# HarryShomer/LPFormer

Hardware: AMD Instinct MI355X
Metric: candidate link-pairs scored/sec (whole node) (higher is better)
Workload: dtype f32

## Files before the change

lpformer_amd/csrc/tail_chain.hip:

```cpp
#include <type_traits>

#include "lpf_common.h"

namespace {

typedef float f32x4 __attribute__((ext_vector_type(4)));

#ifndef LPF_TC_GROUPS
#define LPF_TC_GROUPS 4
#endif
constexpr int TC_GROUPS = LPF_TC_GROUPS;
constexpr int TC_WAVES = 2 * TC_GROUPS;
constexpr int TC_THREADS = 64 * TC_WAVES;

struct TailArgs {
    int64_t M;
    const float *x; int64_t ldx; int KA;
    const float *addend; int64_t ldadd;
    const float *wA, *lnA_g, *lnA_b; int NA;
    const float *tail; int64_t ldtail;
    const float *wB, *bB, *lnB_g, *lnB_b; int NB;
    const float *re; int64_t ldre;
    const float *wC, *bC; int NC;
    const float *wdot, *bdot;
    float *logit, *prob;
    const float *part;
    const float *bnd;
    int64_t units_cap;
    const int32_t *type_ptr;
    const float *att_bias;
    const int64_t *sel_ctl;
    int n_counts;
    const float *rows; int64_t ldrows;
    const int32_t *perm;
    const int64_t *n_full;
    const float *bC_empty;
    const float *row_empty;
    const float *X; int64_t ldX;
    const int64_t *batch; int64_t batch_ld, n_rows;
    const float *wE, *bE, *lnE_g, *lnE_b;
};

constexpr int tc_per_thread(int ntp) { return (ntp * 64 + TC_THREADS - 1) / TC_THREADS; }
constexpr int tc_stage_stride(int ntp) { return (ntp * 64 + 511) / 512 * 512; }

typedef short bf16x4_bits __attribute__((ext_vector_type(4)));
template <int P, int NTP, typename T>
__device__ __forceinline__ void tc_load(T (&r)[P], const float *packed, int stage, int tid) {
    const T *src = reinterpret_cast<const T *>(packed) + (int64_t)stage * tc_stage_stride(NTP);
#pragma unroll
    for (int e = 0; e < P; ++e) {
        const int i = e * TC_THREADS + tid;
#ifdef TC_NOWLOAD
        r[e] = T{};
        (void)src; (void)i;
#else
        r[e] = src[i < tc_stage_stride(NTP) ? i : 0];
#endif
    }
}
template <int P, typename T>
__device__ __forceinline__ void tc_store(const T (&r)[P], T *slab, int tid) {
#pragma unroll
    for (int e = 0; e < P; ++e) slab[e * TC_THREADS + tid] = r[e];
}

#define TC_PIN() __builtin_amdgcn_sched_barrier(0)

template <int TPW>
__device__ __forceinline__ void tc_mfma(f32x4 (&acc)[TPW], const f32x4 *lw, const f32x4 bv, bool last = true) {
    f32x4 a[TPW];
#pragma unroll
    for (int c = 0; c < TPW; ++c) a[c] = lw[c * 64];
#pragma unroll
    for (int u = 0; u < 4; ++u) {
#pragma unroll
        for (int c = 0; c < TPW - 1; ++c) acc[c] = __builtin_amdgcn_mfma_f32_16x16x4f32(a[c][u], bv[u], acc[c], 0, 0, 0);
        if (last) acc[TPW - 1] = __builtin_amdgcn_mfma_f32_16x16x4f32(a[TPW - 1][u], bv[u], acc[TPW - 1], 0, 0, 0);
    }
}
template <int TPW>
__device__ __forceinline__ void tc_mfma(f32x4 (&acc)[TPW], const uint2 *lw, const f32x4 bv, bool last = true) {
    bf16x4_bits b;
#pragma unroll
    for (int u = 0; u < 4; ++u) b[u] = (short)lpf_f32_to_bf16(bv[u]);
#pragma unroll
    for (int c = 0; c < TPW; ++c) {
        if (c == TPW - 1 && !last) break;
        const uint2 w = lw[c * 64];
        const bf16x4_bits a = {(short)(w.x & 0xffffu), (short)(w.x >> 16), (short)(w.y & 0xffffu), (short)(w.y >> 16)};
        acc[c] = __builtin_amdgcn_mfma_f32_16x16x16bf16_1k(a, b, acc[c], 0, 0, 0);
    }
}

constexpr int TC_XCH_SLOT = TC_WAVES * 16;
template <int TPW>
__device__ __forceinline__ void tc_layernorm(f32x4 (&acc)[TPW], int fbase, int n, const float *g, const float *b, int half,
                                             int q, float *my_x, const float *peer_x, bool relu) {
    float s1 = 0.f;
#pragma unroll
    for (int c = 0; c < TPW; ++c) s1 += acc[c][0] + acc[c][1] + acc[c][2] + acc[c][3];
    s1 = lpf_quad_sum(s1);
    if (q == 0) *my_x = s1;
    __syncthreads();
    const float mean = (half == 0 ? s1 + *peer_x : *peer_x + s1) / (float)n;
    float s2 = 0.f;
#pragma unroll
    for (int c = 0; c < TPW; ++c)
#pragma unroll
        for (int r = 0; r < 4; ++r) {
            const float d = (fbase + 16 * c + r < n) ? acc[c][r] - mean : 0.f;
            s2 += d * d;
        }
    s2 = lpf_quad_sum(s2);
    if (q == 0) my_x[TC_XCH_SLOT] = s2;
    __syncthreads();
    const float p2 = peer_x[TC_XCH_SLOT];
    const float rstd = 1.0f / sqrtf((half == 0 ? s2 + p2 : p2 + s2) / (float)n + 1e-5f);
#pragma unroll
    for (int c = 0; c < TPW; ++c) {
        const f32x4 gg = *reinterpret_cast<const f32x4 *>(g + fbase + 16 * c);
        const f32x4 bb = *reinterpret_cast<const f32x4 *>(b + fbase + 16 * c);
        acc[c] = (acc[c] - mean) * rstd * gg + bb;
        if (relu) {
#pragma unroll
            for (int r = 0; r < 4; ++r) acc[c][r] = fmaxf(acc[c][r], 0.f);
        }
    }
}

#ifdef TC_STAMPS
__device__ uint64_t *tc_stamp_buf = nullptr;
#define TC_STAMP(k) do { if (lane == 0) st_t[k] = wall_clock64(); } while (0)
#define TC_STAMPS_OUT(kind) do { if (lane == 0 && tc_stamp_buf) { uint64_t *o__ = tc_stamp_buf + ((int64_t)blockIdx.x * TC_WAVES + wave) * 16; \
        for (int k__ = 0; k__ < 8; ++k__) o__[k__] = st_t[k__]; o__[15] = (kind); } } while (0)
#else
#define TC_STAMP(k) do { } while (0)
#define TC_STAMPS_OUT(kind) do { } while (0)
#endif

template <int NTA, int NTB, int NTC>
struct TcShape {
    static constexpr int NTPA = (NTA + 1) & ~1, NTPB = (NTB + 1) & ~1, NTPC = (NTC + 1) & ~1;
    static constexpr int PA = tc_per_thread(NTPA), PB = tc_per_thread(NTPB), PC = tc_per_thread(NTPC);
    static constexpr int PM = PA > PB ? (PA > PC ? PA : PC) : (PB > PC ? PB : PC);
    static constexpr int SLAB = PM * TC_THREADS;
    static constexpr int HT = NTPA > NTPB ? NTPA : NTPB;
    static constexpr int HID = TC_GROUPS * HT * 64;
    static constexpr int XCH = 5 * TC_WAVES * 16;
    static constexpr int VEC_B = 3 * 16 * NTPA, VEC_C = VEC_B + 3 * 16 * NTPB, VEC_N = VEC_C + 2 * 16 * NTPC;
    static constexpr size_t BYTES = (size_t)(2 * SLAB + HID) * sizeof(f32x4) + (XCH + VEC_N) * sizeof(float);
    static_assert(NTC >= 32 || BYTES <= 81920, "two workgroups share a CU's 160 KB of LDS");
};

template <int NTA, int NTB, int NTC, int WM = 0, bool ROWS = false, bool EW = false>
__global__ __launch_bounds__(TC_THREADS, NTC >= 32 ? 2 : (TC_THREADS >= 512 ? 4 : 3)) void tail_chain_kernel(const TailArgs A) {
    using S = TcShape<NTA, NTB, NTC>;
    constexpr bool WB = WM != 0;
    using WT = typename std::conditional<WM == 1, uint2, f32x4>::type;
    constexpr int NTPA = S::NTPA, NTPB = S::NTPB, NTPC = S::NTPC;
    constexpr int TPWA = NTPA / 2, TPWB = NTPB / 2, TPWC = NTPC / 2;
    constexpr int NGE = NTA;
    extern __shared__ __attribute__((aligned(16))) f32x4 lds[];
    f32x4 *hid = lds + 2 * S::SLAB;
    float *xch = reinterpret_cast<float *>(hid + S::HID);
    const int tid = threadIdx.x, lane = tid & 63, wave = tid >> 6;
    const int grp = wave >> 1, half = wave & 1, q = lane >> 4, j = lane & 15;
    float *my_x = xch + wave * 16 + j;
    const float *peer_x = xch + (wave ^ 1) * 16 + j;
    float *vec = xch + S::XCH;
    f32x4 *my_hid = hid + (grp * S::HT) * 64 + lane;
    int buf = 0;
#ifdef TC_STAMPS
    uint64_t st_t[8] = {0};
    TC_STAMP(0);
#endif

    const int64_t tile = blockIdx.x;
    const int64_t pos = tile * (16 * TC_GROUPS) + grp * 16 + j;
    const bool live = pos < A.M;
    bool lite = false;
    int64_t m = pos;
    if constexpr (ROWS) {
        if (A.perm) {
            m = A.perm[live ? pos : A.M - 1];
            lite = tile * (16 * TC_GROUPS) >= *A.n_full;
        }
    }
    const int64_t mm = live ? m : (ROWS && A.perm ? m : A.M - 1);
    bool no_sel = false;
    if constexpr (ROWS) no_sel = A.perm && A.row_empty && (live ? pos : A.M - 1) >= *A.n_full;

    constexpr int VP0 = EW ? 0 : S::VEC_B / 4, VPN = S::VEC_N / 4 - VP0, VPT = (VPN + TC_THREADS - 1) / TC_THREADS;
    f32x4 vecr[VPT];
#pragma unroll
    for (int e = 0; e < VPT; ++e) {
        int p = VP0 + e * TC_THREADS + tid;
        p = p < S::VEC_N / 4 ? p : S::VEC_N / 4 - 1;
        const float *src;
        if (p >= S::VEC_C / 4) {
            const int o = p - S::VEC_C / 4;
            src = o < 4 * NTPC ? (lite ? A.bC_empty : A.bC) + 4 * o : A.wdot + 4 * (o - 4 * NTPC);
        } else if (!EW || p >= S::VEC_B / 4) {
            const int o = p - S::VEC_B / 4;
            src = o < 4 * NTPB ? A.bB + 4 * o : (o < 8 * NTPB ? A.lnB_g + 4 * (o - 4 * NTPB) : A.lnB_b + 4 * (o - 8 * NTPB));
        } else {
            src = p < 4 * NTPA ? A.bE + 4 * p : (p < 8 * NTPA ? A.lnE_g + 4 * (p - 4 * NTPA) : A.lnE_b + 4 * (p - 8 * NTPA));
        }
        vecr[e] = *reinterpret_cast<const f32x4 *>(src);
    }
    TC_PIN();
    auto tc_vec_publish = [&]() __attribute__((always_inline)) {
#pragma unroll
        for (int e = 0; e < VPT; ++e) {
            int p = VP0 + e * TC_THREADS + tid;
            p = p < S::VEC_N / 4 ? p : S::VEC_N / 4 - 1;
            reinterpret_cast<f32x4 *>(vec)[p] = vecr[e];
        }
    };
    const float *v_bE = vec, *v_lnE_g = vec + 16 * NTPA, *v_lnE_b = vec + 32 * NTPA;
    const float *v_bB = vec + S::VEC_B, *v_lnB_g = v_bB + 16 * NTPB, *v_lnB_b = v_bB + 32 * NTPB;
    const float *v_bC = vec + S::VEC_C, *v_wdot = v_bC + 16 * NTPC;

    f32x4 rowv[ROWS ? TPWA : 1], rowt = (f32x4){0.f, 0.f, 0.f, 0.f};
#pragma unroll
    for (int c = 0; c < (ROWS ? TPWA : 1); ++c) rowv[c] = (f32x4){0.f, 0.f, 0.f, 0.f};
    auto tc_rows_request = [&]() __attribute__((always_inline)) {
        if constexpr (ROWS) {
            const int fbase = 16 * half * TPWA + 4 * q;
            const float *own = A.rows + mm * A.ldrows, *row = no_sel ? A.row_empty : own;
#pragma unroll
            for (int c = 0; c < TPWA; ++c) {
                const int f0 = fbase + 16 * c;
                rowv[c] = *reinterpret_cast<const f32x4 *>(row + (f0 < A.NA ? f0 : 0));
            }
            rowt = *reinterpret_cast<const f32x4 *>(own + A.NA);
        }
    };

    f32x4 accC[TPWC];
    if constexpr (EW) {
        static_assert(ROWS && WM == 0 && S::PA == 1 && NTPA == NTA && NGE % 2 == 0 && 2 * tc_stage_stride(NTPA) <= S::SLAB &&
                          tc_stage_stride(2 * NTPA) == 2 * tc_stage_stride(NTPA), "stage E: the fp32 rows form at D = 128");
        int64_t ra = A.batch[mm], rb = A.batch[A.batch_ld + mm];
        WT wrE[2];
        tc_load<2, 2 * NTPA>(wrE, A.wE, 0, tid);
        TC_PIN();
        if ((uint64_t)ra >= (uint64_t)A.n_rows) ra = 0;
        if ((uint64_t)rb >= (uint64_t)A.n_rows) rb = 0;
        const float *xa = A.X + ra * A.ldX + 4 * q, *xb = A.X + rb * A.ldX + 4 * q;
        f32x4 accE[TPWA];
#pragma unroll
        for (int c = 0; c < TPWA; ++c) accE[c] = (f32x4){0.f, 0.f, 0.f, 0.f};
        f32x4 xra[NGE], xrb[NGE];
#pragma unroll
        for (int kg = 0; kg < NGE; ++kg) {
            xra[kg] = *reinterpret_cast<const f32x4 *>(xa + 16 * kg);
            xrb[kg] = *reinterpret_cast<const f32x4 *>(xb + 16 * kg);
        }
        tc_vec_publish();
#pragma unroll
        for (int kg = 0; kg < NGE; kg += 2) {
            const f32x4 bv0 = xra[kg] * xrb[kg], bv1 = xra[kg + 1] * xrb[kg + 1];
            WT *lw = reinterpret_cast<WT *>(lds) + buf * S::SLAB;
            tc_store<2>(wrE, lw, tid);
            __syncthreads();
            if (kg + 2 < NGE) tc_load<2, 2 * NTPA>(wrE, A.wE, kg / 2 + 1, tid);
            TC_PIN();
            tc_mfma<TPWA>(accE, lw + (half * TPWA) * 64 + lane, bv0);
            tc_mfma<TPWA>(accE, lw + tc_stage_stride(NTPA) + (half * TPWA) * 64 + lane, bv1);
            TC_PIN();
            buf ^= 1;
        }
        if (!lite) tc_rows_request();
        WT wrCe[S::PC];
        tc_load<S::PC, NTPC>(wrCe, A.wC, 0, tid);
        {
            const int fbase = 16 * half * TPWA + 4 * q;
#pragma unroll
            for (int c = 0; c < TPWA; ++c) accE[c] += *reinterpret_cast<const f32x4 *>(v_bE + fbase + 16 * c);
            tc_layernorm<TPWA>(accE, fbase, A.NA, v_lnE_g, v_lnE_b, half, q, my_x, peer_x, true);
#pragma unroll
            for (int c = 0; c < TPWA; ++c) my_hid[(half * TPWA + c) * 64] = accE[c];
        }
        TC_STAMP(7);
#pragma unroll
        for (int c = 0; c < TPWC; ++c) accC[c] = (f32x4){0.f, 0.f, 0.f, 0.f};
#pragma unroll 1
        for (int kg = 0; kg < NGE; ++kg) {
            WT *lw = reinterpret_cast<WT *>(lds) + buf * S::SLAB;
            tc_store<S::PC>(wrCe, lw, tid);
            __syncthreads();
            if (kg + 1 < NGE) tc_load<S::PC, NTPC>(wrCe, A.wC, kg + 1, tid);
            tc_mfma<TPWC>(accC, lw + (half * TPWC) * 64 + lane, my_hid[kg * 64]);
            buf ^= 1;
        }
        TC_STAMP(4);
        if (!lite) __syncthreads();
    }

    if constexpr (ROWS) {
        if (lite) {
            f32x4 (&acc)[TPWC] = accC;
            if constexpr (!EW) {
#pragma unroll
            for (int c = 0; c < TPWC; ++c) acc[c] = (f32x4){0.f, 0.f, 0.f, 0.f};
            WT wr[S::PC];
            const float *rer = A.re + mm * A.ldre + 4 * q;
            tc_load<S::PC, NTPC>(wr, A.wC, 0, tid);
            f32x4 xr = *reinterpret_cast<const f32x4 *>(rer);
            tc_vec_publish();
#pragma unroll 1
            for (int kg = 0; kg < NGE; ++kg) {
                const f32x4 bv = xr;
                WT *lw = reinterpret_cast<WT *>(lds) + buf * S::SLAB;
                tc_store<S::PC>(wr, lw, tid);
                __syncthreads();
                if (kg + 1 < NGE) {
                    tc_load<S::PC, NTPC>(wr, A.wC, kg + 1, tid);
                    xr = *reinterpret_cast<const f32x4 *>(rer + 16 * (kg + 1));
                }
                tc_mfma<TPWC>(acc, lw + (half * TPWC) * 64 + lane, bv);
                buf ^= 1;
            }
            }
            const int fbase = 16 * half * TPWC + 4 * q;
            float d = 0.f;
#pragma unroll
            for (int c = 0; c < TPWC; ++c) {
                const f32x4 b = *reinterpret_cast<const f32x4 *>(v_bC + fbase + 16 * c);
                const f32x4 w = *reinterpret_cast<const f32x4 *>(v_wdot + fbase + 16 * c);
#pragma unroll
                for (int r = 0; r < 4; ++r) d = fmaf(fmaxf(acc[c][r] + b[r], 0.f), w[r], d);
            }
            d = lpf_quad_sum(d);
            if (q == 0) my_x[4 * TC_XCH_SLOT] = d;
            __syncthreads();
            if (live && q == 0 && half == 0) {
                d = d + peer_x[4 * TC_XCH_SLOT] + A.bdot[0];
                if (A.sel_ctl && A.sel_ctl[3] != 0) d = __builtin_nanf("");
                if (A.logit) A.logit[m] = d;
                if (A.prob) A.prob[m] = 1.0f / (1.0f + expf(-d));
            }
            TC_STAMP(6);
            TC_STAMPS_OUT(1);
            return;
        }
    }
    if constexpr (!EW) tc_vec_publish();
    f32x4 accA[TPWA];
#pragma unroll
    for (int c = 0; c < TPWA; ++c) accA[c] = (f32x4){0.f, 0.f, 0.f, 0.f};
    int seg_cnt[3] = {0, 0, 0};
    if (!WB && !ROWS && A.part == nullptr) {
        const float *xa = A.x + mm * A.ldx;
        const int ngA = (A.KA + 15) >> 4;
        f32x4 wr[S::PA];
        tc_load<S::PA, NTPA>(wr, A.wA, 0, tid);
        int kk = 4 * q < A.KA ? 4 * q : A.KA - 4;
        f32x4 xr = *reinterpret_cast<const f32x4 *>(xa + kk);
#pragma unroll 1
        for (int kg = 0; kg < ngA; ++kg) {
            const f32x4 bv = (16 * kg + 4 * q < A.KA) ? xr : (f32x4){0.f, 0.f, 0.f, 0.f};
            f32x4 *lw = lds + buf * S::SLAB;
            tc_store<S::PA>(wr, lw, tid);
            __syncthreads();
            if (kg + 1 < ngA) {
                tc_load<S::PA, NTPA>(wr, A.wA, kg + 1, tid);
                kk = 16 * (kg + 1) + 4 * q;
                kk = kk < A.KA ? kk : A.KA - 4;
                xr = *reinterpret_cast<const f32x4 *>(xa + kk);
            }
            tc_mfma<TPWA>(accA, lw + (half * TPWA) * 64 + lane, bv);
            buf ^= 1;
        }
    }
    WT wrB[S::PB];
    tc_load<S::PB, NTPB>(wrB, A.wB, 0, tid);
    if constexpr (ROWS) {
        const int fbase = 16 * half * TPWA + 4 * q;
        if constexpr (!EW) tc_rows_request();
#pragma unroll
        for (int c = 0; c < TPWA; ++c) accA[c] = fbase + 16 * c < A.NA ? rowv[c] : (f32x4){0.f, 0.f, 0.f, 0.f};
    } else if (A.part == nullptr) {
        const int fbase = 16 * half * TPWA + 4 * q;
        f32x4 ad[TPWA];
#pragma unroll
        for (int c = 0; c < TPWA; ++c) {
            const int f0 = fbase + 16 * c;
            ad[c] = *reinterpret_cast<const f32x4 *>(A.addend + mm * A.ldadd + (f0 < A.NA ? f0 : 0));
        }
#pragma unroll
        for (int c = 0; c < TPWA; ++c) accA[c] += (fbase + 16 * c < A.NA) ? ad[c] : (f32x4){0.f, 0.f, 0.f, 0.f};
    } else {
        const int fbase = 16 * half * TPWA + 4 * q;
        const int64_t rs = A.NA + 4;
        float mx = -INFINITY, den = 0.f;
        f32x4 v[TPWA];
#pragma unroll
        for (int c = 0; c < TPWA; ++c) v[c] = (f32x4){0.f, 0.f, 0.f, 0.f};
        auto fetch = [&](const float *rec, f32x4 &h, f32x4 *b) __attribute__((always_inline)) {
            h = *reinterpret_cast<const f32x4 *>(rec + A.NA);
#pragma unroll
            for (int c = 0; c < TPWA; ++c) {
                const int f0 = fbase + 16 * c;
                b[c] = *reinterpret_cast<const f32x4 *>(rec + (f0 < A.NA ? f0 : 0));
            }
        };
        auto merge = [&](const f32x4 &h, const f32x4 *b) __attribute__((always_inline)) {
            const float mn = fmaxf(mx, h[0]);
            const float sa = __expf(mx - mn), sb = __expf(h[0] - mn);
            den = fmaf(den, sa, h[1] * sb);
#pragma unroll
            for (int c = 0; c < TPWA; ++c) v[c] = v[c] * sa + b[c] * sb;
            mx = mn;
        };
        int lo[3], hi[3], n_p[3];
#pragma unroll
        for (int t = 0; t < 3; ++t) {
            const int32_t *tp = A.type_ptr + (int64_t)t * (A.M + 1) + mm;
            lo[t] = tp[0];
            hi[t] = tp[1];
        }
        {
            f32x4 h0[3], b0[3][TPWA];
#pragma unroll
            for (int t = 0; t < 3; ++t) {
                seg_cnt[t] = hi[t] - lo[t];
                const bool some = hi[t] > lo[t] && ((hi[t] - 1) >> 4) < A.units_cap;
                n_p[t] = some ? ((hi[t] - 1) >> 4) - (lo[t] >> 4) + 1 : 0;
                const float *rec = n_p[t] > 1 ? A.bnd + ((((int64_t)t * A.units_cap + (lo[t] >> 4)) * 2) + 1) * rs
                                              : A.part + ((int64_t)t * A.M + mm) * rs;
                h0[t] = (f32x4){0.f, 0.f, 0.f, 0.f};
#pragma unroll
                for (int c = 0; c < TPWA; ++c) b0[t][c] = (f32x4){0.f, 0.f, 0.f, 0.f};
                if (n_p[t] > 0) fetch(rec, h0[t], b0[t]);
            }
#pragma unroll
            for (int t = 0; t < 3; ++t)
                if (n_p[t] > 0) merge(h0[t], b0[t]);
        }
        const int r0 = n_p[0] > 1 ? n_p[0] - 1 : 0, r1 = n_p[1] > 1 ? n_p[1] - 1 : 0, r2 = n_p[2] > 1 ? n_p[2] - 1 : 0;
        const int n_rest = r0 + r1 + r2;
        constexpr int NB = TPWA >= 4 ? 2 : 4;
#pragma unroll 1
        for (int k0 = 0; k0 < n_rest; k0 += NB) {
            f32x4 hh[NB], bb[NB][TPWA];
#pragma unroll
            for (int i = 0; i < NB; ++i) {
                const int k = k0 + i < n_rest ? k0 + i : n_rest - 1;
                const int t = k < r0 ? 0 : (k < r0 + r1 ? 1 : 2);
                const int jj = k - (t == 0 ? 0 : (t == 1 ? r0 : r0 + r1));
                const int ut = t == 0 ? lo[0] >> 4 : (t == 1 ? lo[1] >> 4 : lo[2] >> 4);
                fetch(A.bnd + (((int64_t)t * A.units_cap + ut + 1 + jj) * 2) * rs, hh[i], bb[i]);
            }
#pragma unroll
            for (int i = 0; i < NB; ++i)
                if (k0 + i < n_rest) merge(hh[i], bb[i]);
        }
        const float inv = 1.0f / (den + 1e-16f);
#pragma unroll
        for (int c = 0; c < TPWA; ++c) {
            const int f0 = fbase + 16 * c;
            if (f0 < A.NA) accA[c] = v[c] * inv + *reinterpret_cast<const f32x4 *>(A.att_bias + f0);
        }
    }
    {
        const int fbase = 16 * half * TPWA + 4 * q;
        if constexpr (!ROWS) tc_layernorm<TPWA>(accA, fbase, A.NA, A.lnA_g, A.lnA_b, half, q, my_x, peer_x, false);
#pragma unroll
        for (int c = 0; c < TPWA; ++c) my_hid[(half * TPWA + c) * 64] = accA[c];
    }

    TC_STAMP(1);
    f32x4 accB[TPWB];
#pragma unroll
    for (int c = 0; c < TPWB; ++c) accB[c] = (f32x4){0.f, 0.f, 0.f, 0.f};
    {
        f32x4 tailv = (f32x4){0.f, 0.f, 0.f, 0.f};
        if constexpr (ROWS) {
            if (q == 0 && !no_sel) tailv = rowt;
        } else if (q == 0) {
            if (A.part == nullptr) {
                tailv = *reinterpret_cast<const f32x4 *>(A.tail + mm * A.ldtail);
            } else {
                const float n0 = (float)seg_cnt[0], n1 = (float)seg_cnt[1], n2 = (float)seg_cnt[2];
                tailv = A.n_counts == 4 ? (f32x4){n0, n1, n2, n0 + n1}
                                         : (A.n_counts == 3 ? (f32x4){n0, n1, n0 + n1, 0.f} : (f32x4){n0, 0.f, 0.f, 0.f});
            }
        }
#pragma unroll
        for (int kg = 0; kg < NTPA + 1; ++kg) {
            WT *lw = reinterpret_cast<WT *>(lds) + buf * S::SLAB;
            tc_store<S::PB>(wrB, lw, tid);
            __syncthreads();
            if (kg + 1 < NTPA + 1) tc_load<S::PB, NTPB>(wrB, A.wB, kg + 1, tid);
            const f32x4 bv = kg < NTPA ? my_hid[(kg < NTPA ? kg : 0) * 64] : tailv;
            tc_mfma<TPWB>(accB, lw + (half * TPWB) * 64 + lane, bv, !((NTB & 1) && half == 1));
            buf ^= 1;
        }
    }
    TC_STAMP(2);
    WT wrC[S::PC];
    tc_load<S::PC, NTPC>(wrC, A.wC, EW ? NGE : 0, tid);
    const float *rer = EW ? nullptr : A.re + mm * A.ldre + 4 * q;
    f32x4 xr = (f32x4){0.f, 0.f, 0.f, 0.f};
    if constexpr (!EW) xr = *reinterpret_cast<const f32x4 *>(rer);
    {
        const int fbase = 16 * half * TPWB + 4 * q;
#pragma unroll
        for (int c = 0; c < TPWB; ++c) accB[c] += *reinterpret_cast<const f32x4 *>(v_bB + fbase + 16 * c);
        tc_layernorm<TPWB>(accB, fbase, A.NB, v_lnB_g, v_lnB_b, half, q, my_x + 2 * TC_XCH_SLOT, peer_x + 2 * TC_XCH_SLOT, true);
#pragma unroll
        for (int c = 0; c < TPWB; ++c) my_hid[(half * TPWB + c) * 64] = accB[c];
    }

    TC_STAMP(3);
    if constexpr (!EW) {
#pragma unroll
    for (int c = 0; c < TPWC; ++c) accC[c] = (f32x4){0.f, 0.f, 0.f, 0.f};
#pragma unroll 1
    for (int kg = 0; kg < NGE; ++kg) {
        const f32x4 bv = xr;
        WT *lw = reinterpret_cast<WT *>(lds) + buf * S::SLAB;
        tc_store<S::PC>(wrC, lw, tid);
        __syncthreads();
        tc_load<S::PC, NTPC>(wrC, A.wC, kg + 1, tid);
        if (kg + 1 < NGE) xr = *reinterpret_cast<const f32x4 *>(rer + 16 * (kg + 1));
        tc_mfma<TPWC>(accC, lw + (half * TPWC) * 64 + lane, bv);
        buf ^= 1;
    }
    TC_STAMP(4);
    }
#pragma unroll
    for (int kg = 0; kg < NTB; ++kg) {
        WT *lw = reinterpret_cast<WT *>(lds) + buf * S::SLAB;
        tc_store<S::PC>(wrC, lw, tid);
        __syncthreads();
        if (kg + 1 < NTB) tc_load<S::PC, NTPC>(wrC, A.wC, NGE + kg + 1, tid);
        TC_PIN();
        tc_mfma<TPWC>(accC, lw + (half * TPWC) * 64 + lane, my_hid[kg * 64]);
        TC_PIN();
        buf ^= 1;
    }
    TC_STAMP(5);
    {
        const int fbase = 16 * half * TPWC + 4 * q;
        float d = 0.f;
#pragma unroll
        for (int c = 0; c < TPWC; ++c) {
            const f32x4 b = *reinterpret_cast<const f32x4 *>(v_bC + fbase + 16 * c);
            const f32x4 w = *reinterpret_cast<const f32x4 *>(v_wdot + fbase + 16 * c);
#pragma unroll
            for (int r = 0; r < 4; ++r) d = fmaf(fmaxf(accC[c][r] + b[r], 0.f), w[r], d);
        }
        d = lpf_quad_sum(d);
        if (q == 0) my_x[4 * TC_XCH_SLOT] = d;
        __syncthreads();
        if (live && q == 0 && half == 0) {
            d = d + peer_x[4 * TC_XCH_SLOT] + A.bdot[0];
            if (A.sel_ctl && A.sel_ctl[3] != 0) d = __builtin_nanf("");
            if (A.logit) A.logit[m] = d;
            if (A.prob) A.prob[m] = 1.0f / (1.0f + expf(-d));
        }
    }
    TC_STAMP(6);
    TC_STAMPS_OUT(0);
}

template <int NTA, int NTB, int NTC, int WM = 0, bool ROWS = false, bool EW = false>
int tc_launch(const TailArgs &a, hipStream_t s) {
    constexpr size_t lds = TcShape<NTA, NTB, NTC>::BYTES;
    auto kern = tail_chain_kernel<NTA, NTB, NTC, WM, ROWS, EW>;
    LPF_SET_MAX_LDS(kern, lds);
    const int64_t blocks = (a.M + 16 * TC_GROUPS - 1) / (16 * TC_GROUPS);
    if (blocks > 0x7fffffff) return LPF_ERR_UNSUPPORTED;
    hipLaunchKernelGGL(kern, dim3((unsigned)blocks), dim3(TC_THREADS), lds, s, a);
    LPF_CHECK_LAUNCH();
    return LPF_OK;
}

}

#ifdef TC_STAMPS
extern "C" int lpf_tail_chain_set_stamps(void *buf) {
    return hipMemcpyToSymbol(HIP_SYMBOL(tc_stamp_buf), &buf, sizeof(buf)) == hipSuccess ? LPF_OK : LPF_ERR_LAUNCH;
}
#endif


extern "C" int lpf_tail_chain_f32(int64_t M, int32_t D, int32_t n_counts, const float *G, int64_t ldg,
                                  const float *wA_packed, const float *lnA_g, const float *lnA_b, const float *counts,
                                  int64_t ldc, const float *wB_packed, const float *bB, const float *lnB_g,
                                  const float *lnB_b, const float *r_e, int64_t ldre, const float *wC_packed,
                                  const float *bC, const float *w_dot, const float *b_dot, float *logit, float *prob,
                                  void *stream) {
    if (M == 0) return LPF_OK;
    LPF_REQUIRE(M > 0 && G && wA_packed && lnA_g && lnA_b && counts && wB_packed && bB && lnB_g && lnB_b && r_e &&
                wC_packed && bC && w_dot && b_dot && (logit || prob));
    LPF_REQUIRE(n_counts >= 1 && n_counts <= 4 && (ldg & 3) == 0 && ldg >= 4 * D + 4 && (ldc & 3) == 0 && ldc >= 4 &&
                (ldre & 3) == 0 && ldre >= D);
    LPF_REQUIRE(lpf_aligned16(G) && lpf_aligned16(counts) && lpf_aligned16(r_e) && lpf_aligned16(wA_packed) &&
                lpf_aligned16(wB_packed) && lpf_aligned16(wC_packed) && lpf_aligned16(lnA_g) && lpf_aligned16(lnA_b) &&
                lpf_aligned16(bB) && lpf_aligned16(lnB_g) && lpf_aligned16(lnB_b) && lpf_aligned16(bC) &&
                lpf_aligned16(w_dot));
    TailArgs a{M, G + D, ldg, 3 * D + 4, G, ldg, wA_packed, lnA_g, lnA_b, D, counts, ldc, wB_packed, bB, lnB_g,
               lnB_b, D + n_counts, r_e, ldre, wC_packed, bC, 2 * D, w_dot, b_dot, logit, prob,
               nullptr, nullptr, 0, nullptr, nullptr, nullptr, n_counts, nullptr, 0, nullptr, nullptr, nullptr, nullptr};
    hipStream_t s = static_cast<hipStream_t>(stream);
    switch (D) {
        case 32: return tc_launch<2, 3, 4>(a, s);
        case 64: return tc_launch<4, 5, 8>(a, s);
        case 128: return tc_launch<8, 9, 16>(a, s);
        default: return LPF_ERR_UNSUPPORTED;
    }
}

extern "C" int lpf_tail_chain_merge_f32(int64_t M, int32_t D, int32_t n_counts, const float *part, const float *bnd,
                                        int64_t units_cap, const int32_t *type_ptr, const float *att_bias, const float *lnA_g,
                                        const float *lnA_b, const float *wB_packed, const float *bB, const float *lnB_g,
                                        const float *lnB_b, const float *r_e, int64_t ldre, const float *wC_packed,
                                        const float *bC, const float *w_dot, const float *b_dot,
                                        const int64_t *sel_ctl, float *logit, float *prob, void *stream) {
    if (M == 0) return LPF_OK;
    LPF_REQUIRE(M > 0 && part && bnd && units_cap > 0 && lpf_aligned16(bnd) && type_ptr && att_bias && lnA_g && lnA_b && wB_packed && bB && lnB_g && lnB_b && r_e &&
                wC_packed && bC && w_dot && b_dot && (logit || prob));
    LPF_REQUIRE((n_counts == 1 || n_counts == 3 || n_counts == 4) && (ldre & 3) == 0 && ldre >= D);
    LPF_REQUIRE(lpf_aligned16(part) && lpf_aligned16(att_bias) && lpf_aligned16(r_e) && lpf_aligned16(wB_packed) &&
                lpf_aligned16(wC_packed) && lpf_aligned16(lnA_g) && lpf_aligned16(lnA_b) && lpf_aligned16(bB) &&
                lpf_aligned16(lnB_g) && lpf_aligned16(lnB_b) && lpf_aligned16(bC) && lpf_aligned16(w_dot));
    TailArgs a{M, nullptr, 0, 0, nullptr, 0, nullptr, lnA_g, lnA_b, D, nullptr, 0, wB_packed, bB, lnB_g,
               lnB_b, D + n_counts, r_e, ldre, wC_packed, bC, 2 * D, w_dot, b_dot, logit, prob,
               part, bnd, units_cap, type_ptr, att_bias, sel_ctl, n_counts, nullptr, 0, nullptr, nullptr, nullptr, nullptr};
    hipStream_t s = static_cast<hipStream_t>(stream);
    switch (D) {
        case 32: return tc_launch<2, 3, 4>(a, s);
        case 64: return tc_launch<4, 5, 8>(a, s);
        case 128: return tc_launch<8, 9, 16>(a, s);
        default: return LPF_ERR_UNSUPPORTED;
    }
}

extern "C" int lpf_tail_chain_merge_bf16(int64_t M, int32_t D, int32_t n_counts, const float *part, const float *bnd,
                                         int64_t units_cap, const int32_t *type_ptr, const float *att_bias,
                                         const float *lnA_g, const float *lnA_b, const void *wB_packed_bf16,
                                         const float *bB, const float *lnB_g, const float *lnB_b, const float *r_e,
                                         int64_t ldre, const void *wC_packed_bf16, const float *bC, const float *w_dot,
                                         const float *b_dot, const int64_t *sel_ctl, float *logit, float *prob,
                                         void *stream) {
    if (M == 0) return LPF_OK;
    LPF_REQUIRE(M > 0 && part && bnd && units_cap > 0 && lpf_aligned16(bnd) && type_ptr && att_bias && lnA_g && lnA_b &&
                wB_packed_bf16 && bB && lnB_g && lnB_b && r_e && wC_packed_bf16 && bC && w_dot && b_dot &&
                (logit || prob));
    LPF_REQUIRE((n_counts == 1 || n_counts == 3 || n_counts == 4) && (ldre & 3) == 0 && ldre >= D);
    LPF_REQUIRE(lpf_aligned16(part) && lpf_aligned16(att_bias) && lpf_aligned16(r_e) && lpf_aligned16(wB_packed_bf16) &&
                lpf_aligned16(wC_packed_bf16) && lpf_aligned16(lnA_g) && lpf_aligned16(lnA_b) && lpf_aligned16(bB) &&
                lpf_aligned16(lnB_g) && lpf_aligned16(lnB_b) && lpf_aligned16(bC) && lpf_aligned16(w_dot));
    TailArgs a{M, nullptr, 0, 0, nullptr, 0, nullptr, lnA_g, lnA_b, D, nullptr, 0,
               static_cast<const float *>(wB_packed_bf16), bB, lnB_g, lnB_b, D + n_counts, r_e, ldre,
               static_cast<const float *>(wC_packed_bf16), bC, 2 * D, w_dot, b_dot, logit, prob,
               part, bnd, units_cap, type_ptr, att_bias, sel_ctl, n_counts, nullptr, 0, nullptr, nullptr, nullptr, nullptr};
    hipStream_t s = static_cast<hipStream_t>(stream);
    switch (D) {
        case 32: return tc_launch<2, 3, 4, 1>(a, s);
        case 64: return tc_launch<4, 5, 8, 1>(a, s);
        case 128: return tc_launch<8, 9, 16, 1>(a, s);
        default: return LPF_ERR_UNSUPPORTED;
    }
}

namespace {
template <int WM>
int tc_rows(int64_t M, int32_t D, int32_t n_counts, const float *rows, int64_t ldrows, const void *wB, const float *bB,
            const float *lnB_g, const float *lnB_b, const float *r_e, int64_t ldre, const void *wC, const float *bC,
            const float *w_dot, const float *b_dot, const int64_t *sel_ctl, float *logit, float *prob, void *stream,
            const int32_t *perm = nullptr, const int64_t *n_full = nullptr, const float *bC_empty = nullptr,
            const float *row_empty = nullptr) {
    if (M == 0) return LPF_OK;
    LPF_REQUIRE(!perm || (n_full && bC_empty && lpf_aligned16(bC_empty)));
    LPF_REQUIRE(!row_empty || (perm && lpf_aligned16(row_empty)));
    LPF_REQUIRE(M > 0 && rows && wB && bB && lnB_g && lnB_b && r_e && wC && bC && w_dot && b_dot && (logit || prob));
    LPF_REQUIRE((n_counts == 1 || n_counts == 3 || n_counts == 4) && (ldre & 3) == 0 && ldre >= D && (ldrows & 3) == 0 &&
                ldrows >= D + 4);
    LPF_REQUIRE(lpf_aligned16(rows) && lpf_aligned16(r_e) && lpf_aligned16(wB) && lpf_aligned16(wC) && lpf_aligned16(bB) &&
                lpf_aligned16(lnB_g) && lpf_aligned16(lnB_b) && lpf_aligned16(bC) && lpf_aligned16(w_dot));
    TailArgs a{M, nullptr, 0, 0, nullptr, 0, nullptr, nullptr, nullptr, D, nullptr, 0, static_cast<const float *>(wB), bB,
               lnB_g, lnB_b, D + n_counts, r_e, ldre, static_cast<const float *>(wC), bC, 2 * D, w_dot, b_dot, logit, prob,
               nullptr, nullptr, 0, nullptr, nullptr, sel_ctl, n_counts, rows, ldrows, perm, n_full, bC_empty, row_empty};
    hipStream_t s = static_cast<hipStream_t>(stream);
    switch (D) {
        case 32: return tc_launch<2, 3, 4, WM, true>(a, s);
        case 64: return tc_launch<4, 5, 8, WM, true>(a, s);
        case 128: return tc_launch<8, 9, 16, WM, true>(a, s);
        case 256: return tc_launch<16, 17, 32, WM, true>(a, s);
        default: return LPF_ERR_UNSUPPORTED;
    }
}
}

extern "C" int lpf_tail_chain_rows_f32(int64_t M, int32_t D, int32_t n_counts, const float *rows, int64_t ldrows,
                                       const float *wB_packed, const float *bB, const float *lnB_g, const float *lnB_b,
                                       const float *r_e, int64_t ldre, const float *wC_packed, const float *bC,
                                       const float *w_dot, const float *b_dot, const int64_t *sel_ctl, float *logit,
                                       float *prob, void *stream) {
    return tc_rows<0>(M, D, n_counts, rows, ldrows, wB_packed, bB, lnB_g, lnB_b, r_e, ldre, wC_packed, bC, w_dot, b_dot,
                          sel_ctl, logit, prob, stream);
}

extern "C" int lpf_tail_chain_rows_bf16(int64_t M, int32_t D, int32_t n_counts, const float *rows, int64_t ldrows,
                                        const void *wB_packed_bf16, const float *bB, const float *lnB_g, const float *lnB_b,
                                        const float *r_e, int64_t ldre, const void *wC_packed_bf16, const float *bC,
                                        const float *w_dot, const float *b_dot, const int64_t *sel_ctl, float *logit,
                                        float *prob, void *stream) {
    return tc_rows<1>(M, D, n_counts, rows, ldrows, wB_packed_bf16, bB, lnB_g, lnB_b, r_e, ldre, wC_packed_bf16, bC, w_dot,
                         b_dot, sel_ctl, logit, prob, stream);
}

extern "C" int lpf_tail_chain_rows_perm_f32(int64_t M, int32_t D, int32_t n_counts, const float *rows, int64_t ldrows,
                                            const float *wB_packed, const float *bB, const float *lnB_g,
                                            const float *lnB_b, const float *r_e, int64_t ldre, const float *wC_packed,
                                            const float *bC, const float *w_dot, const float *b_dot,
                                            const int64_t *sel_ctl, const int32_t *perm, const int64_t *n_full,
                                            const float *bC_empty, const float *row_empty, float *logit, float *prob,
                                            void *stream) {
    LPF_REQUIRE(perm && n_full && bC_empty);
    return tc_rows<0>(M, D, n_counts, rows, ldrows, wB_packed, bB, lnB_g, lnB_b, r_e, ldre, wC_packed, bC, w_dot, b_dot,
                          sel_ctl, logit, prob, stream, perm, n_full, bC_empty, row_empty);
}

extern "C" int lpf_tail_chain_rows_perm_bf16(int64_t M, int32_t D, int32_t n_counts, const float *rows, int64_t ldrows,
                                             const void *wB_packed_bf16, const float *bB, const float *lnB_g,
                                             const float *lnB_b, const float *r_e, int64_t ldre,
                                             const void *wC_packed_bf16, const float *bC, const float *w_dot,
                                             const float *b_dot, const int64_t *sel_ctl, const int32_t *perm,
                                             const int64_t *n_full, const float *bC_empty, const float *row_empty,
                                             float *logit, float *prob, void *stream) {
    LPF_REQUIRE(perm && n_full && bC_empty);
    return tc_rows<1>(M, D, n_counts, rows, ldrows, wB_packed_bf16, bB, lnB_g, lnB_b, r_e, ldre, wC_packed_bf16, bC, w_dot,
                         b_dot, sel_ctl, logit, prob, stream, perm, n_full, bC_empty, row_empty);
}

extern "C" int lpf_tail_chain_rows_perm_ew_f32(int64_t M, int32_t D, int32_t n_counts, const float *rows, int64_t ldrows,
                                               const float *wB_packed, const float *bB, const float *lnB_g,
                                               const float *lnB_b, const float *r_e, int64_t ldre, const float *wC_packed,
                                               const float *bC, const float *w_dot, const float *b_dot,
                                               const int64_t *sel_ctl, const int32_t *perm, const int64_t *n_full,
                                               const float *bC_empty, const float *row_empty, const float *X, int64_t ldx,
                                               const int64_t *batch, int64_t batch_ld, int64_t n_rows,
                                               const float *wE_packed, const float *bE, const float *lnE_g,
                                               const float *lnE_b, float *logit, float *prob, void *stream) {
    if (!wE_packed)
        return lpf_tail_chain_rows_perm_f32(M, D, n_counts, rows, ldrows, wB_packed, bB, lnB_g, lnB_b, r_e, ldre, wC_packed, bC,
                                            w_dot, b_dot, sel_ctl, perm, n_full, bC_empty, row_empty, logit, prob, stream);
    if (M == 0) return LPF_OK;
    if (D != 128) return LPF_ERR_UNSUPPORTED;
    LPF_REQUIRE(perm && n_full && bC_empty && lpf_aligned16(bC_empty) && (!row_empty || lpf_aligned16(row_empty)));
    LPF_REQUIRE(M > 0 && rows && wB_packed && bB && lnB_g && lnB_b && wC_packed && bC && w_dot && b_dot && (logit || prob));
    LPF_REQUIRE((n_counts == 1 || n_counts == 3 || n_counts == 4) && (ldrows & 3) == 0 && ldrows >= D + 4);
    LPF_REQUIRE(X && batch && bE && lnE_g && lnE_b && n_rows > 0 && batch_ld >= M && (ldx & 3) == 0 && ldx >= D);
    LPF_REQUIRE(lpf_aligned16(rows) && lpf_aligned16(wB_packed) && lpf_aligned16(wC_packed) && lpf_aligned16(bB) &&
                lpf_aligned16(lnB_g) && lpf_aligned16(lnB_b) && lpf_aligned16(bC) && lpf_aligned16(w_dot) &&
                lpf_aligned16(X) && lpf_aligned16(wE_packed) && lpf_aligned16(bE) && lpf_aligned16(lnE_g) &&
                lpf_aligned16(lnE_b));
    TailArgs a{M, nullptr, 0, 0, nullptr, 0, nullptr, nullptr, nullptr, D, nullptr, 0, wB_packed, bB,
               lnB_g, lnB_b, D + n_counts, nullptr, 0, wC_packed, bC, 2 * D, w_dot, b_dot, logit, prob,
               nullptr, nullptr, 0, nullptr, nullptr, sel_ctl, n_counts, rows, ldrows, perm, n_full, bC_empty, row_empty,
               X, ldx, batch, batch_ld, n_rows, wE_packed, bE, lnE_g, lnE_b};
    return tc_launch<8, 9, 16, 0, true, true>(a, static_cast<hipStream_t>(stream));
}
```

Measured before the change: 274.3 million.

## Split stage E row gathers across wave halves and exchange products via LDS

Stage E used to have each of the two paired waves load the full gathered X rows for its 16 pairs, so every row was fetched twice. Now each half-wave pair loads only half the row chunks, using 32-byte-strided lanes that cover 8 chunks per pair. It forms the elementwise products and writes them into the group's hidden LDS tiles with padded strides. The MFMA loop then reads its B operands from LDS, which halves global gather traffic and register use at the cost of extra LDS stores and loads. Timing stamps for the row-load and stage-E end are also added under TC_STAMPS.

```diff
diff --git a/lpformer_amd/csrc/tail_chain.hip b/lpformer_amd/csrc/tail_chain.hip
--- a/lpformer_amd/csrc/tail_chain.hip
+++ b/lpformer_amd/csrc/tail_chain.hip
@@ -133,8 +133,10 @@
 __device__ uint64_t *tc_stamp_buf = nullptr;
 #define TC_STAMP(k) do { if (lane == 0) st_t[k] = wall_clock64(); } while (0)
 #define TC_STAMPS_OUT(kind) do { if (lane == 0 && tc_stamp_buf) { uint64_t *o__ = tc_stamp_buf + ((int64_t)blockIdx.x * TC_WAVES + wave) * 16; \
-        for (int k__ = 0; k__ < 8; ++k__) o__[k__] = st_t[k__]; o__[15] = (kind); } } while (0)
+        for (int k__ = 0; k__ < 10; ++k__) o__[k__] = st_t[k__]; o__[15] = (kind); } } while (0)
+#define TC_STAMP_ROWS() do { __builtin_amdgcn_s_waitcnt(0x0f70); TC_STAMP(8); } while (0)
 #else
+#define TC_STAMP_ROWS() do { } while (0)
 #define TC_STAMP(k) do { } while (0)
 #define TC_STAMPS_OUT(kind) do { } while (0)
 #endif
@@ -172,7 +174,7 @@
     f32x4 *my_hid = hid + (grp * S::HT) * 64 + lane;
     int buf = 0;
 #ifdef TC_STAMPS
-    uint64_t st_t[8] = {0};
+    uint64_t st_t[10] = {0};
     TC_STAMP(0);
 #endif
 
@@ -242,36 +244,50 @@
     if constexpr (EW) {
         static_assert(ROWS && WM == 0 && S::PA == 1 && NTPA == NTA && NGE % 2 == 0 && 2 * tc_stage_stride(NTPA) <= S::SLAB &&
                           tc_stage_stride(2 * NTPA) == 2 * tc_stage_stride(NTPA), "stage E: the fp32 rows form at D = 128");
-        int64_t ra = A.batch[mm], rb = A.batch[A.batch_ld + mm];
+        constexpr int TE_KG = 68, TE_Q2 = 34;
+        static_assert((NGE - 1) * TE_KG + TE_Q2 + 32 <= S::HT * 64, "stage E's product tiles fit a group's hidden tiles");
+        const int gj = 8 * half + (lane >> 3), gp = lane & 7;
+        const int64_t gpos = tile * (16 * TC_GROUPS) + grp * 16 + gj;
+        const int64_t gm = gpos < A.M ? gpos : A.M - 1;
+        const int64_t gmm = A.perm ? A.perm[gm] : gm;
+        int64_t ra = A.batch[gmm], rb = A.batch[A.batch_ld + gmm];
         WT wrE[2];
         tc_load<2, 2 * NTPA>(wrE, A.wE, 0, tid);
         TC_PIN();
         if ((uint64_t)ra >= (uint64_t)A.n_rows) ra = 0;
         if ((uint64_t)rb >= (uint64_t)A.n_rows) rb = 0;
-        const float *xa = A.X + ra * A.ldX + 4 * q, *xb = A.X + rb * A.ldX + 4 * q;
+        const float *xa = A.X + ra * A.ldX + 4 * gp, *xb = A.X + rb * A.ldX + 4 * gp;
         f32x4 accE[TPWA];
 #pragma unroll
         for (int c = 0; c < TPWA; ++c) accE[c] = (f32x4){0.f, 0.f, 0.f, 0.f};
-        f32x4 xra[NGE], xrb[NGE];
-#pragma unroll
-        for (int kg = 0; kg < NGE; ++kg) {
-            xra[kg] = *reinterpret_cast<const f32x4 *>(xa + 16 * kg);
-            xrb[kg] = *reinterpret_cast<const f32x4 *>(xb + 16 * kg);
+        f32x4 xra[NGE / 2], xrb[NGE / 2];
+#pragma unroll
+        for (int i = 0; i < NGE / 2; ++i) {
+            xra[i] = *reinterpret_cast<const f32x4 *>(xa + 32 * i);
+            xrb[i] = *reinterpret_cast<const f32x4 *>(xb + 32 * i);
         }
         tc_vec_publish();
+        TC_STAMP_ROWS();
+        {
+            f32x4 *pe = hid + (grp * S::HT) * 64 + (gp >> 2) * TE_KG + ((gp >> 1) & 1) * TE_Q2 + (gp & 1) * 16 + gj;
+#pragma unroll
+            for (int i = 0; i < NGE / 2; ++i) pe[2 * i * TE_KG] = xra[i] * xrb[i];
+        }
+        const f32x4 *my_pe = hid + (grp * S::HT) * 64 + (q >> 1) * TE_Q2 + (q & 1) * 16 + j;
 #pragma unroll
         for (int kg = 0; kg < NGE; kg += 2) {
-            const f32x4 bv0 = xra[kg] * xrb[kg], bv1 = xra[kg + 1] * xrb[kg + 1];
             WT *lw = reinterpret_cast<WT *>(lds) + buf * S::SLAB;
             tc_store<2>(wrE, lw, tid);
             __syncthreads();
             if (kg + 2 < NGE) tc_load<2, 2 * NTPA>(wrE, A.wE, kg / 2 + 1, tid);
             TC_PIN();
+            const f32x4 bv0 = my_pe[kg * TE_KG], bv1 = my_pe[(kg + 1) * TE_KG];
             tc_mfma<TPWA>(accE, lw + (half * TPWA) * 64 + lane, bv0);
             tc_mfma<TPWA>(accE, lw + tc_stage_stride(NTPA) + (half * TPWA) * 64 + lane, bv1);
             TC_PIN();
             buf ^= 1;
         }
+        TC_STAMP(9);
         if (!lite) tc_rows_request();
         WT wrCe[S::PC];
         tc_load<S::PC, NTPC>(wrCe, A.wC, 0, tid);
```

Measured after the change: 278.1 million, median of 6. 1.01x the previous value.
